# data61/gossamer

Measured on AMD Instinct MI355X. Metric: M k-mers/s (canonical, counted) at k=25, 150 bp reads, higher is better.
Workload: dtype u64

## Files before the change

### gossamer_amd/csrc/fused_path.hpp

```cpp
#pragma once

enum { kFusedDeclined = 0, kFusedDone = 1, kFusedNeedFull = 2, kFusedGoOn = -1, kFusedAgain = -2 };
constexpr uint32_t kFusedGrid = 256 * GOSS_E1_OCC;
#ifndef GOSS_FUSED_NKEYS2
#define GOSS_FUSED_NKEYS2 14
#endif
#ifndef GOSS_FUSED_GRID2
#define GOSS_FUSED_GRID2 512
#endif
constexpr uint32_t kFusedGrid2 = GOSS_FUSED_GRID2;
constexpr double kValidSlackA = 1.06, kValidSlackB = 1.17;
constexpr uint64_t kValidSizingMin = 640u << 20;

struct FusedForm {
    enum Table {
        kSmall,
        kBig,
        kWide,
        k96,
        kRem32
    };
    Table table = kSmall;
    uint32_t segbits = kSegBits;
    bool msd = false;
// ... 516 lines not shown
    out->n = n; out->tiles = tiles; out->windows = hp->windows;
    return kFusedGoOn;
}

struct FusedLookback { LookbackCtl* ctl; LookbackCtl* hctl; };

inline int count_rem32(const FusedChunk<Key1>& ch, FusedForm form, const Sub32Regions& sub, const FirstLevelResult& fl, const GapTable* dgt,
                       FusedLookback lb, Run* r)
{
    goss_gpu_ctx* c = ch.c;
    Key1* ka = ch.ka; Key1* kb = ch.kb;
    const uint64_t n = fl.n, tiles = fl.tiles;
    const uint32_t r32_regions = form.r32_regions(), r32_bits = form.r32_bits, r32_split = form.r32_split, rbits32 = form.rbits32;
    const uint32_t sqbit32 = c->len - 1;
    const bool narrow = form.narrow, squeeze = form.squeeze;
    SubTable32* dsub = (SubTable32*)c->arena.temp(sizeof(SubTable32));
    unsigned long long* cur2 = (unsigned long long*)c->arena.temp((uint64_t)r32_regions * 4);
    uint64_t* seg_beg = (uint64_t*)c->arena.temp((uint64_t)r32_regions * 8);
    uint64_t* seg_end = (uint64_t*)c->arena.temp((uint64_t)r32_regions * 8);
    Tile32* tdesc = (Tile32*)c->arena.temp(std::max<uint64_t>(tiles, 1) * sizeof(Tile32));
    HIP_TRY(hipMemcpyAsync(dsub->start, sub.start.data(), (uint64_t)r32_regions * 8, hipMemcpyHostToDevice, c->stream));
    HIP_TRY(hipMemcpyAsync(dsub->cap, sub.cap.data(), (uint64_t)r32_regions * 4, hipMemcpyHostToDevice, c->stream));
    HIP_TRY(hipMemsetAsync(cur2, 0, (uint64_t)r32_regions * 4, c->stream));
    if (narrow && r32_bits == 9)
        hipLaunchKernelGGL(HIP_KERNEL_NAME(tiles32_kernel<Sub32N<9>::kTileSlots>), dim3(grid_for(tiles, 256)), dim3(256), 0, c->stream,
                           dgt, tdesc, (uint32_t)tiles);
    else if (narrow)
        hipLaunchKernelGGL(HIP_KERNEL_NAME(tiles32_kernel<Sub32N<10>::kTileSlots>), dim3(grid_for(tiles, 256)), dim3(256), 0, c->stream,
                           dgt, tdesc, (uint32_t)tiles);
    else
        hipLaunchKernelGGL(HIP_KERNEL_NAME(tiles32_kernel<kSub32Tile>), dim3(grid_for(tiles, 256)), dim3(256), 0, c->stream,
                           dgt, tdesc, (uint32_t)tiles);
    {
        PhaseTimer t(c, GOSS_T_SCATTER, n);
        const dim3 g2((uint32_t)((tiles + 7) / 8 * 8));
#define GOSS_LAUNCH_S32N(SQ, B2, NRW)                                                                                    \
    hipLaunchKernelGGL(HIP_KERNEL_NAME(subpart32_kernel<SQ, B2, NRW>), g2, dim3(kTB), 0, c->stream, (const Key1*)ka, (uint32_t*)kb, rbits32, \
                       sqbit32, cur2, (const Tile32*)tdesc, (uint32_t)tiles, (const SubTable32*)dsub, lb.ctl)
#define GOSS_LAUNCH_S32(SQ, B2) do { if (narrow) GOSS_LAUNCH_S32N(SQ, B2, true); else GOSS_LAUNCH_S32N(SQ, B2, false); } while (0)
        if (squeeze) GOSS_LAUNCH_S32(true, 9);
        else if (r32_bits == 9) GOSS_LAUNCH_S32(false, 9);
        else GOSS_LAUNCH_S32(false, 10);
#undef GOSS_LAUNCH_S32
#undef GOSS_LAUNCH_S32N
        t.stop();
    }
    hipLaunchKernelGGL(sub_bounds32_kernel, dim3(r32_regions / 256), dim3(256), 0, c->stream, (const SubTable32*)dsub,
                       (const uint32_t*)cur2, r32_regions, seg_beg, seg_end);
    HIP_TRY(hipMemcpyAsync(lb.hctl, lb.ctl, sizeof(LookbackCtl), hipMemcpyDeviceToHost, c->stream));
    HIP_TRY(hipStreamSynchronize(c->stream));
    if (lb.hctl->error) { c->fused_overflows++; return ch.decline("a 32-bit sub-region overflowed"); }
    ch.lap("second level (32-bit remainders)");
    const uint32_t* rems = (const uint32_t*)kb;
    Key1* spare32 = ka;
    uint32_t nseg32 = r32_regions;
    if (r32_split)
    {
        nseg32 = r32_regions << r32_split;
        uint64_t* sub_beg = (uint64_t*)c->arena.temp((uint64_t)nseg32 * 8);
// ... 1 lines not shown
        {
            PhaseTimer t(c, GOSS_T_SCATTER, n);
            hipLaunchKernelGGL(subsplit32_kernel, unit_grid(r32_regions), dim3(kTB), 0, c->stream, (const uint32_t*)kb, (uint32_t*)ka,
                               (const uint64_t*)seg_beg, (const uint64_t*)seg_end, rbits32 - (squeeze ? 1u : 0u), r32_split, sub_beg, sub_end);
            t.stop();
        }
        check_launch("third-level split kernel");
        seg_beg = sub_beg; seg_end = sub_end;
        rems = (const uint32_t*)ka;
        spare32 = kb;
        ch.lap("third level (sub-segments)");
    }
    int rc;
    for (;;)
    {
        rc = segment_reduce32(c, rems, spare32, n, r, seg_beg, seg_end, form.r32_slots, squeeze, rbits32, sqbit32, nseg32, r32_split);
        if (rc != 1 || form.r32_slots >= 16384 || c->rem32_slots) break;
        c->segment_retries++;
        form = form.larger_r32_table();
    }
    if (rc != 0)
    {
        c->segment_retries++;
        if (rc == 1 && r32_split < (uint32_t)kSub32SplitMax) c->rem32_split_min = r32_split + 1;
        else c->rem32 = false;
        if (c->debug) std::fprintf(stderr, "libgossgpu: fused path: 32-bit form with %u + %u bits overflowed (%d), redoing the chunk %s\n", r32_bits, r32_split, rc,
                                   c->rem32 ? "with more sub-segments" : "in the 8-byte form");
        return kFusedAgain;
    }
    c->fused_msd_chunks++;
    c->rem32_chunks++;
// ... 238 lines not shown
```

### gossamer_amd/csrc/goss_gpu.hip

```cpp
#include "../../include/goss_gpu.h"

#include <hip/hip_runtime.h>
#include <dlfcn.h>

#include <algorithm>
#include <chrono>
#include <cmath>
#include <cstdio>
#include <cstdlib>
#include <cstring>
#include <functional>
#include <map>
#include <mutex>
#include <string>
#include <system_error>
#include <thread>
#include <vector>

#include "goss_kernels.hpp"
#include "goss_reader.hpp"

using namespace goss;

namespace {
// ... 1015 lines not shown
    HIP_TRY(hipMemcpyAsync(seg_dst, seg_cnt, (uint64_t)nunit * 8, hipMemcpyDeviceToDevice, c->stream));
    exclusive_scan_u64(c, seg_dst, nunit);
    out->m = m;
    out->keys = c->arena.perm(std::max<uint64_t>(m, 1) * sizeof(K));
    out->counts = (uint32_t*)c->arena.perm(std::max<uint64_t>(m, 1) * 4);
    hipLaunchKernelGGL(HIP_KERNEL_NAME(seg_gather_kernel<K>), unit_grid(nunit), dim3(kTB), 0, c->stream,
                       (const K*)stage_keys, (const uint32_t*)stage_counts, (const uint64_t*)seg_pos,
                       (const uint64_t*)seg_dst, (const uint64_t*)seg_cnt, (K*)out->keys, out->counts);
    t.stop();
    HIP_TRY(hipStreamSynchronize(c->stream));
    c->arena.release(mark);
    return 0;
}

int segment_reduce32(goss_gpu_ctx* c, const uint32_t* rems, Key1* spare, uint64_t n, Run* out, const uint64_t* seg_beg,
                     const uint64_t* seg_end, int slots, bool squeeze, uint32_t rbits, uint32_t sqbit, uint32_t nseg, uint32_t split_bits)
{
    uint64_t mark = c->arena.mark();
    PhaseTimer t(c, GOSS_T_REDUCE, n);
    uint64_t* seg_pos = (uint64_t*)c->arena.temp((uint64_t)nseg * 8);
    uint64_t* seg_cnt = (uint64_t*)c->arena.temp(((uint64_t)nseg + 1) * 8);
    uint64_t* seg_dst = (uint64_t*)c->arena.temp(((uint64_t)nseg + 1) * 8);
    SegOut* so = (SegOut*)c->arena.temp(sizeof(SegOut));
    const uint64_t cap = n * sizeof(Key1) / (sizeof(Key1) + 4);
    Key1* stage_keys = spare;
    uint32_t* stage_counts = (uint32_t*)(spare + cap);
    SegOut hso{};
    hso.stage_cap = cap;
    HIP_TRY(hipMemcpyAsync(so, &hso, sizeof(SegOut), hipMemcpyHostToDevice, c->stream));
#define GOSS_LAUNCH_R32(SLOTS, SQ)                                                                                       \
    hipLaunchKernelGGL(HIP_KERNEL_NAME(seg_hash_reduce32b_kernel<SLOTS, SQ>), unit_grid(nseg), dim3(SLOTS <= 4096 ? kTB : SLOTS / 4096 * kTB), 0, c->stream, rems, seg_beg, \
                       seg_end, so, seg_pos, seg_cnt, stage_keys, stage_counts, rbits, sqbit, split_bits)
    if (slots == 2048) { if (squeeze) GOSS_LAUNCH_R32(2048, true); else GOSS_LAUNCH_R32(2048, false); }
    else if (slots == 8192) { if (squeeze) GOSS_LAUNCH_R32(8192, true); else GOSS_LAUNCH_R32(8192, false); }
    else if (slots == 16384) { if (squeeze) GOSS_LAUNCH_R32(16384, true); else GOSS_LAUNCH_R32(16384, false); }
    else { if (squeeze) GOSS_LAUNCH_R32(4096, true); else GOSS_LAUNCH_R32(4096, false); }
#undef GOSS_LAUNCH_R32
    check_launch("32-bit segment counting kernel");
    SegOut* h = (SegOut*)c->h_pinned;
    HIP_TRY(hipMemcpyAsync(h, so, sizeof(SegOut), hipMemcpyDeviceToHost, c->stream));
    HIP_TRY(hipStreamSynchronize(c->stream));
#if defined(GOSS_STAMPS)
    if (h->stamps[7])
        std::fprintf(stderr, "libgossgpu: counting stamps per segment (cycles of wave 0): set-up %.0f  loads+copy %.0f  fast path %.0f  slow path %.0f  closing barrier %.0f  ordering %.0f  write-out %.0f   (%llu segments)\n",
                     (double)h->stamps[0] / h->stamps[7], (double)h->stamps[1] / h->stamps[7], (double)h->stamps[2] / h->stamps[7], (double)h->stamps[3] / h->stamps[7],
                     (double)h->stamps[4] / h->stamps[7], (double)h->stamps[5] / h->stamps[7], (double)h->stamps[6] / h->stamps[7], (unsigned long long)h->stamps[7]);
#endif
    if (h->overflow == 1u && c->overflow_by_sort)
    {
        SegOut hs = *h;
        const int rc = count_overflowed_units<Key1>(c, nseg, seg_beg, seg_end, seg_pos, seg_cnt, &hs, stage_keys, stage_counts,
            [&](uint32_t u, uint64_t first, uint64_t cnt_u, Key1* dst) {
                const uint64_t prefix = (uint64_t)(u >> split_bits) << rbits;
                if (squeeze)
                    hipLaunchKernelGGL(HIP_KERNEL_NAME(expand_rem32_kernel<true>), dim3(grid_for(cnt_u, kTB)), dim3(kTB), 0, c->stream, rems + first, cnt_u, prefix, sqbit, dst);
                else
                    hipLaunchKernelGGL(HIP_KERNEL_NAME(expand_rem32_kernel<false>), dim3(grid_for(cnt_u, kTB)), dim3(kTB), 0, c->stream, rems + first, cnt_u, prefix, sqbit, dst);
            },
            [&](uint32_t u) -> Key1 {
                const uint32_t rem_bits = rbits - (squeeze ? 1u : 0u);
                const uint32_t sub = split_bits ? (u & ((1u << split_bits) - 1u)) << (rem_bits - split_bits) : 0u;
                const uint64_t low = squeeze ? rem32_unpack<true>(sub, sqbit) : rem32_unpack<false>(sub, sqbit);
                return Key1{((uint64_t)(u >> split_bits) << rbits) | low};
            });
        *h = hs;
        if (rc == 2) h->overflow = 2u;
    }
    if (h->overflow)
    {
        const int why = (h->overflow & 1u) ? 1 : 2;
        t.stop();
        c->arena.release(mark);
// ... 3988 lines not shown
```

### gossamer_amd/csrc/kernels_count.hpp

```cpp
#pragma once
#include <type_traits>

#include <hip/hip_runtime.h>
#include <stdint.h>

#include "goss_key.hpp"
#include "kernels_partition.hpp"

namespace goss {


constexpr int kSegBits = 16;
constexpr int kSegBitsMax = 24;
constexpr int kSegSlots = 4096;
constexpr int kSegLimit = 3072;
constexpr int kSegSlots2 = 2048;
constexpr int kSegLimit2 = 1536;

template <class K>
__global__ void seg_bounds_kernel(const K* __restrict__ keys, uint64_t n, uint32_t shift, uint32_t nseg,
                                  uint64_t* __restrict__ seg_off)
{
    uint32_t s = blockIdx.x * blockDim.x + threadIdx.x;
    if (s > nseg) return;
// ... 6 lines not shown
    seg_off[s] = a;
}

struct SegOut {
    unsigned long long cursor;
    uint32_t overflow;
    uint32_t count_overflow;
    unsigned long long stage_cap;
#if defined(GOSS_STAMPS)
    unsigned long long stamps[8];
#endif
};

constexpr unsigned long long kSegOverflowed = ~0ULL;

template <bool SQ>
__global__ __launch_bounds__(kTB) void expand_rem32_kernel(const uint32_t* __restrict__ rems, uint64_t n, uint64_t prefix, uint32_t sqbit,
                                                           Key1* __restrict__ out)
{
    const uint64_t i = (uint64_t)blockIdx.x * kTB + threadIdx.x;
    if (i < n) out[i].lo = prefix | rem32_unpack<SQ>(rems[i], sqbit);
}
__global__ __launch_bounds__(kTB) void expand_rem96_kernel(const Rem96* __restrict__ recs, uint64_t n, uint64_t seg, uint32_t rem_bits,
                                                           Key2* __restrict__ out)
{
    const uint64_t i = (uint64_t)blockIdx.x * kTB + threadIdx.x;
    if (i >= n) return;
    const Rem96 r = recs[i];
    const unsigned __int128 full = ((unsigned __int128)seg << rem_bits) | ((unsigned __int128)r.r2 << 64) | ((uint64_t)r.r0 | ((uint64_t)r.r1 << 32));
    out[i] = Key2{(uint64_t)full, (uint64_t)(full >> 64)};
}

template <class K>
__global__ __launch_bounds__(kTB) void unit_bounds_kernel(const K* __restrict__ keys, uint64_t m, const K* __restrict__ lows, const K* __restrict__ highs,
                                                          const uint8_t* __restrict__ last, const uint32_t* __restrict__ units, uint32_t nunits,
                                                          unsigned long long cursor, uint64_t* __restrict__ seg_pos, uint64_t* __restrict__ seg_cnt)
// ... 433 lines not shown
                                                                             uint32_t rem_bits, uint32_t round_bits)
{
    (void)round_bits;
    seg_hash_reduce_body<kSegBigThreads, kSegBigSlots, false>(keys, seg_off, seg_end, so, seg_pos, seg_cnt, stage_keys, stage_counts, rem_bits, 0u);
}

__global__ __launch_bounds__(kSegBigThreads) void seg_hash_reduce_shared_kernel(const Key1* __restrict__ keys, const uint64_t* __restrict__ seg_off,
                                                                                const uint64_t* __restrict__ seg_end, SegOut* __restrict__ so,
                                                                                uint64_t* __restrict__ seg_pos, uint64_t* __restrict__ seg_cnt,
                                                                                Key1* __restrict__ stage_keys, uint32_t* __restrict__ stage_counts,
                                                                                uint32_t rem_bits, uint32_t round_bits)
{
    seg_hash_reduce_body<kSegBigThreads, kSegBigSlots, true>(keys, seg_off, seg_end, so, seg_pos, seg_cnt, stage_keys, stage_counts, rem_bits, round_bits);
}

constexpr uint32_t kR32Mul = 0x9E3779B1u, kR32MulInv = 0x0E8B2F51u;
__host__ __device__ __forceinline__ uint32_t r32_mix(uint32_t k) { return (k ^ (k >> 15)) * kR32Mul; }
__host__ __device__ __forceinline__ uint32_t r32_unmix(uint32_t f) { const uint32_t y = f * kR32MulInv; return y ^ (y >> 15) ^ (y >> 30); }

__device__ __forceinline__ uint32_t r32b_slot_offset(const uint32_t __attribute__((ext_vector_type(4)))& q, uint32_t k)
{
    uint32_t off;
    unsigned long long m0, m1, m2, m3;
    asm("v_cmp_eq_u32_e64 %1, %5, %9\n\t"
        "v_cmp_eq_u32_e64 %2, %6, %9\n\t"
        "v_cmp_eq_u32_e64 %3, %7, %9\n\t"
        "v_cmp_eq_u32_e64 %4, %8, %9\n\t"
        "v_cndmask_b32_e64 %0, 16, 12, %1\n\t"
        "v_cndmask_b32_e64 %0, %0, 8, %2\n\t"
        "v_cndmask_b32_e64 %0, %0, 4, %3\n\t"
        "v_cndmask_b32_e64 %0, %0, 0, %4"
        : "=&v"(off), "=&s"(m0), "=&s"(m1), "=&s"(m2), "=&s"(m3)
        : "v"(q.w), "v"(q.z), "v"(q.y), "v"(q.x), "v"(k));
// ... 8 lines not shown
        "v_cmp_lt_u32_e64 %6, 15, %10\n\t"
        "v_cmp_lt_u32_e64 %7, 15, %11\n\t"
        "v_cndmask_b32_e64 %0, %0, %12, %4\n\t"
        "v_cndmask_b32_e64 %1, %1, %12, %5\n\t"
        "v_cndmask_b32_e64 %2, %2, %12, %6\n\t"
        "v_cndmask_b32_e64 %3, %3, %12, %7"
        : "+v"(t[0]), "+v"(t[1]), "+v"(t[2]), "+v"(t[3]), "=&s"(m0), "=&s"(m1), "=&s"(m2), "=&s"(m3)
        : "v"(off[0]), "v"(off[1]), "v"(off[2]), "v"(off[3]), "v"(dummy));
}

#ifndef GOSS_R32B_VEC
#define GOSS_R32B_VEC 4
#endif
template <int SLOTS> struct R32bCfg { static constexpr int kThreads = SLOTS <= 4096 ? kTB : SLOTS == 8192 ? 2 * kTB : 4 * kTB;
                                      static constexpr int kOcc = SLOTS == 2048 ? 5 : SLOTS == 4096 ? 4 : SLOTS == 8192 ? 2 : 1; };
template <int SLOTS, bool SQ>
__global__ __launch_bounds__(R32bCfg<SLOTS>::kThreads, R32bCfg<SLOTS>::kOcc) void seg_hash_reduce32b_kernel(const uint32_t* __restrict__ rems, const uint64_t* __restrict__ seg_off,
                                                                const uint64_t* __restrict__ seg_end, SegOut* __restrict__ so,
                                                                uint64_t* __restrict__ seg_pos, uint64_t* __restrict__ seg_cnt,
                                                                Key1* __restrict__ stage_keys, uint32_t* __restrict__ stage_counts,
                                                                uint32_t rbits, uint32_t sqbit, uint32_t split_bits)
{
    constexpr int NT = R32bCfg<SLOTS>::kThreads;
    constexpr int kLimit = SLOTS / 4 * 3;
    constexpr int BB = SLOTS == 16384 ? 12 : SLOTS == 8192 ? 11 : SLOTS == 4096 ? 10 : SLOTS == 2048 ? 9 : -1;
    constexpr uint32_t NB = SLOTS / 4;
    constexpr uint32_t kCnt = 4u * SLOTS;
    static_assert(BB > 0, "table size");
    __shared__ __attribute__((aligned(16))) unsigned long long tab[SLOTS + 32];
    __shared__ uint32_t ndist, ovf;
    __shared__ unsigned long long sh_base;
// ... 11 lines not shown
        return;
    }
    if (e - b > 0xFFFFFFF0ULL)
    {
        if (tid == 0) { atomicOr(&so->overflow, 2u); seg_pos[s] = 0; seg_cnt[s] = 0; }
        return;
    }
    typedef uint32_t u32x4 __attribute__((ext_vector_type(4)));
    typedef __attribute__((address_space(3))) uint8_t* lds_bytes;
    typedef const __attribute__((address_space(3))) u32x4* lds_bucket_plain;
    typedef const volatile __attribute__((address_space(3))) u32x4* lds_bucket_ptr;
    typedef __attribute__((address_space(3))) uint32_t* lds_word;
    const lds_bytes tb = (lds_bytes)tab;
    uint32_t* const tkey = reinterpret_cast<uint32_t*>(tab);
    uint32_t* const tcnt = tkey + SLOTS;
    auto marker = [](uint32_t bkt) -> uint32_t { return r32_unmix(((bkt ^ 1u) << (32 - BB)) | (3u << (32 - 2 * BB))); };
    for (uint32_t i = tid; i < NB; i += NT)
    {
        const uint32_t m = marker(i);
        *(__attribute__((address_space(3))) u32x4*)(tb + 16 * i) = u32x4{m, m, m, m};
        *(__attribute__((address_space(3))) u32x4*)(tb + kCnt + 16 * i) = u32x4{0u, 0u, 0u, 0u};
    }
    if (tid < 32) tab[SLOTS + tid] = 0;
    if (tid == 0) { ndist = 0; ovf = 0; }
    __syncthreads();
    GOSS_STAMP(0);

    lds_vu32 vovf = (lds_vu32)&ovf;
    const uint32_t dummy = 8u * (uint32_t)SLOTS + 4u * (tid & 63u);
    auto home_of = [](uint32_t f) -> uint32_t { return f >> (32 - BB); };
    auto second_of = [](uint32_t f, uint32_t h) -> uint32_t { return h ^ (((f >> (32 - 2 * BB)) & (NB - 1u)) | 1u); };

    constexpr int kVec = GOSS_R32B_VEC;
    const uint32_t head = (uint32_t)(b & 3ULL);
    const u32x4* const v4 = reinterpret_cast<const u32x4*>(rems + (b - head));
    const uint32_t n = (uint32_t)(e - b) + head;
    const uint32_t nvec = (n + 3u) >> 2, nfull = n >> 2;
    u32x4 nxt[kVec];
#pragma unroll
    for (int u = 0; u < kVec; ++u)
    {
        const uint32_t i = (uint32_t)u * NT + tid;
        nxt[u] = __builtin_nontemporal_load(&v4[i < nvec ? i : nvec - 1]);
    }
    for (uint32_t i0 = 0; i0 < nvec; i0 += (uint32_t)NT * kVec)
    {
// ... 3 lines not shown
#pragma unroll
        for (int u = 0; u < kVec; ++u)
        {
            const uint32_t i = i0 + (uint32_t)(kVec + u) * NT + tid;
            nxt[u] = __builtin_nontemporal_load(&v4[i < nvec ? i : nvec - 1]);
        }
        GOSS_STAMP(1);
        auto four_keys = [&](const u32x4& v, uint32_t live, auto whole_tag) -> uint32_t {
            constexpr bool kWhole = decltype(whole_tag)::value;
            const uint32_t kk[4] = {v.x, v.y, v.z, v.w};
            uint32_t f[4], a1[4], off[4];
            u32x4 q[4];
#pragma unroll
            for (int j = 0; j < 4; ++j)
            {
                f[j] = r32_mix(kk[j]);
                a1[j] = home_of(f[j]) << 4;
                q[j] = *(lds_bucket_plain)(tb + a1[j]);
            }
#pragma unroll
            for (int j = 0; j < 4; ++j) off[j] = r32b_slot_offset(q[j], kk[j]);
            uint32_t t[4];
#pragma unroll
            for (int j = 0; j < 4; ++j)
            {
                t[j] = kCnt + a1[j] + off[j];
                bool miss = off[j] == 16u;
                if (!kWhole) miss = miss && ((live >> j) & 1u);
                if (__builtin_expect(__ballot(miss) != 0, 0))
                {
                    if (miss)
                    {
// ... 17 lines not shown
                __hip_atomic_fetch_add((lds_word)(tb + t[j]), 1u, __ATOMIC_RELAXED, __HIP_MEMORY_SCOPE_WORKGROUP);
                left |= (off[j] & 16u) << j;
            }
            return left >> 4;
        };
        auto slow_keys = [&](const u32x4& v, uint32_t pd) {
            uint32_t key = 0, bk = 0, f = 0, st = 0, moves = 0;
            bool busy = false;
            for (;;)
            {
                if (!busy && pd)
                {
                    const uint32_t j = __ffs(pd) - 1;
                    pd &= pd - 1;
                    key = j == 0 ? v.x : j == 1 ? v.y : j == 2 ? v.z : v.w;
                    f = r32_mix(key);
                    bk = home_of(f);
                    st = 0;
                    busy = true;
                }
                if (!__ballot(busy)) break;
                if (busy)
                {
                    const u32x4 q = *(lds_bucket_ptr)(tb + 16u * bk);
                    const uint32_t mk = marker(bk);
                    const u32x4 qq = u32x4{q.x, q.y, q.z, q.w};
                    const uint32_t ho = r32b_slot_offset(qq, key);
                    const uint32_t eo = r32b_slot_offset(qq, mk);
                    uint32_t hit = ~0u;
                    if (key != mk && ho < 16u) hit = 4 * bk + (ho >> 2);
                    else if (key != mk && eo < 16u)
                    {
// ... 43 lines not shown
    __syncthreads();
    GOSS_STAMP(4);
    if (ovf)
    {
        if (tid == 0) { atomicOr(&so->overflow, 1u); seg_pos[s] = 0; seg_cnt[s] = kSegOverflowed; }
        return;
    }

    constexpr int kPer = SLOTS / NT;
    constexpr int kBins = SLOTS / 4, kBinsPer = kBins / NT, kBinBits = BB;
    __shared__ uint32_t bins[kBins];
    __shared__ uint32_t sh_scan2[NT / 64 + 1];
    __shared__ uint32_t big;
    unsigned long long ck[kPer];
#pragma unroll
    for (int j = 0; j < kPer; ++j) ck[j] = ((unsigned long long)tcnt[tid * kPer + j] << 32) | tkey[tid * kPer + j];
    for (uint32_t i = tid; i < kBins; i += NT) bins[i] = 0;
    if (tid == 0) big = 0;
    __syncthreads();
    const uint32_t rem_bits = rbits - (SQ ? 1u : 0u);
    const uint32_t bsh = rem_bits > (uint32_t)kBinBits + split_bits ? rem_bits - split_bits - kBinBits : 0;
    uint32_t rnk[kPer];
#pragma unroll
    for (int j = 0; j < kPer; ++j)
        if ((ck[j] >> 32) != 0) rnk[j] = atomicAdd(&bins[((uint32_t)ck[j] >> bsh) & (kBins - 1)], 1u);
    __syncthreads();
    uint32_t bn[kBinsPer], bs[kBinsPer], mine = 0;
#pragma unroll
    for (int q = 0; q < kBinsPer; ++q) { bn[q] = bins[tid * kBinsPer + q]; mine += bn[q]; }
    uint32_t tot_occ;
    uint32_t at = block_excl_scan_n<uint32_t, NT / 64>(mine, sh_scan2, &tot_occ);
// ... 737 lines not shown
```

### gossamer_amd/csrc/kernels_extract.hpp

```cpp
#pragma once
#include <type_traits>

#include <hip/hip_runtime.h>
#include <stdint.h>

#include "goss_key.hpp"
#include "kernels_common.hpp"

namespace goss {


struct ExtractCounters {
    unsigned long long keys_out;
    unsigned long long windows;
    unsigned long long hist[512];
};

template <bool PACKED = false>
__global__ __launch_bounds__(kTB) void nonbase_sample_kernel(const uint8_t* __restrict__ aligned, uint64_t nslices,
                                                             uint64_t stride, uint32_t slice,
                                                             unsigned long long* __restrict__ out)
{
    unsigned long long bad = 0, seen = 0;
    for (uint64_t s = blockIdx.x; s < nslices; s += gridDim.x)
// ... 784 lines not shown
                    if (MODE == 0 && REPK == 1)
                    {
                        const uint32_t sel = (uint32_t)__builtin_amdgcn_sbfe((int32_t)flo, len - 1u, 1u);
                        kreg[i].lo = ((uint64_t)bit_select(sel, rhi, fhi) << 32) | bit_select(sel, rlo, flo);
                    }
                    else emit(i, ((uint64_t)fhi << 32) | flo, ((uint64_t)rhi << 32) | rlo);
                    if (i + 1 < P)
                    {
                        r_s2 += 2u;
                        if (r_s2 >= r_nw2 && r_at < 511) next_rec();
                    }
                }
            }
            else if constexpr (FAST)
            {
                const uint32_t kmhi = (uint32_t)(kmask >> 32);
                const uint32_t cw0 = ~(uint32_t)blo, cw1 = ~(uint32_t)(blo >> 32), cw2 = ~(uint32_t)bhi;
                const uint32_t pn = bits - 2;
                const uint32_t nx = (uint32_t)((blo >> pn) | (bhi << (64 - pn)));
                const uint32_t mid = (uint32_t)(blo >> (len - 1));
                const uint64_t f0 = rev64(blo & kmask) >> (64 - bits);
                uint32_t flo = (uint32_t)f0, fhi = (uint32_t)(f0 >> 32);
#pragma unroll
                for (int i = 0; i < P; ++i)
                {
                    if (i)
                    {
                        const uint32_t nb = (nx >> (2 * i)) & 3u;
                        fhi = __builtin_amdgcn_alignbit(fhi, flo, 30) & kmhi;
                        flo = (flo << 2) | nb;
                    }
                    const uint32_t rlo = i ? __builtin_amdgcn_alignbit(cw1, cw0, 2 * i) : cw0;
                    const uint32_t rhi = (i ? __builtin_amdgcn_alignbit(cw2, cw1, 2 * i) : cw1) & kmhi;
                    if (MODE == 0 && REPK == 1)
                    {
                        const uint32_t sel = (uint32_t)__builtin_amdgcn_sbfe((int32_t)mid, 2 * i, 1);
                        kreg[i].lo = ((uint64_t)bit_select(sel, rhi, fhi) << 32) | bit_select(sel, rlo, flo);
                    }
                    else emit(i, ((uint64_t)fhi << 32) | flo, ((uint64_t)rhi << 32) | rlo);
#pragma unroll
                    for (int u = 0; u < S; ++u) rank_key(i * S + u);
                }
            }
            else
            {
                uint64_t f = rev64(blo & kmask) >> (64 - bits);
                uint64_t r = (~blo) & kmask;
                const uint32_t top = bits - 2;
// ... 153 lines not shown
#endif
        {
            uint32_t tb[NK];
#pragma unroll
            for (int i = 0; i < NK; ++i) tb[i] = *reinterpret_cast<const uint32_t*>(reinterpret_cast<const char*>(tab) + bin4[i]);
            if constexpr (NARROW)
            {
                auto put = [&](auto sq_tag, auto hi_tag) {
                    constexpr bool kSq = decltype(sq_tag)::value, kHi = decltype(hi_tag)::value;
                    const uint32_t lomask = kSq ? (1u << nr_sqbit) - 1u : (nr_rbits >= 32 ? 0xFFFFFFFFu : (1u << nr_rbits) - 1u);
                    const uint32_t dbits = (uint32_t)__popc(nr_dmask);
#pragma unroll
                    for (int i = 0; i < NK; ++i)
                    {
                        const uint32_t klo = (uint32_t)kreg[i].lo, khi = (uint32_t)(kreg[i].lo >> 32);
                        uint32_t rem = klo & lomask;
                        if (kSq) rem |= __builtin_amdgcn_alignbit(khi, klo, nr_sqbit + 1u) << nr_sqbit;
                        const uint32_t dg = kHi ? __builtin_amdgcn_ubfe(khi, nr_rbits - 32u, dbits)
                                                : (__builtin_amdgcn_alignbit(khi, klo, nr_rbits) & nr_dmask);
                        const uint32_t la = tb[i] + (rk[i] << 2);
                        *reinterpret_cast<uint32_t*>(lds_all + la) = rem;
                        *reinterpret_cast<uint16_t*>(lds_all + kDigBase + (la >> 1)) = (uint16_t)dg;
                    }
                };
                if (nr_sqbit) { if (nr_rbits >= 32) put(std::true_type{}, std::true_type{}); else put(std::true_type{}, std::false_type{}); }
                else { if (nr_rbits >= 32) put(std::false_type{}, std::true_type{}); else put(std::false_type{}, std::false_type{}); }
            }
            else
#pragma unroll
            for (int i = 0; i < NK; ++i)
            {
                *reinterpret_cast<Key1*>(reinterpret_cast<char*>(sorted) + (tb[i] + (rk[i] << 3))) = kreg[i];
                if (NH > 0)
                {
// ... 736 lines not shown
```

### gossamer_amd/csrc/kernels_partition.hpp

```cpp
#pragma once

#include <hip/hip_runtime.h>
#include <stdint.h>

#include "goss_key.hpp"
#include "kernels_common.hpp"

namespace goss {


#ifndef GOSS_SORT_ITEMS1
#define GOSS_SORT_ITEMS1 32
#endif
#ifndef GOSS_SORT_ITEMS2
#define GOSS_SORT_ITEMS2 16
#endif
#ifndef GOSS_LB_BATCH
#define GOSS_LB_BATCH 1
#endif
template <class K> struct SubCfg {
    static constexpr int kItems = sizeof(K) == 8 ? 22 : 11;
    static constexpr int kTile = 256 * kItems;
};

// ... 458 lines not shown
        K k = stage[i];
        uint64_t o = global_base[key_digit(k, digit)] + i;
        keys_out[o] = k;
        if (HAS_VAL) vals_out[o] = vstage[i];
    }
}

constexpr int kSub32BitsMin = 9, kSub32BitsMax = 10;
constexpr int kSub32SplitMax = 4;
constexpr uint32_t kSub32RegionsMax = 256u << kSub32BitsMax;
struct SubTable32 {
    unsigned long long start[kSub32RegionsMax];
    uint32_t cap[kSub32RegionsMax];
};

template <bool SQ>
__host__ __device__ __forceinline__ uint32_t rem32_pack(uint64_t key, uint32_t rbits, uint32_t sqbit)
{
    const uint64_t x = key & ((1ULL << rbits) - 1ULL);
    if (!SQ) return (uint32_t)x;
    return (uint32_t)(((x >> (sqbit + 1)) << sqbit) | (x & ((1ULL << sqbit) - 1ULL)));
}
template <bool SQ>
__host__ __device__ __forceinline__ uint64_t rem32_unpack(uint32_t r, uint32_t sqbit)
{
    if (!SQ) return r;
    return (((uint64_t)r >> sqbit) << (sqbit + 1)) | ((uint64_t)r & ((1ULL << sqbit) - 1ULL));
}

struct Tile32 { unsigned long long base; uint32_t n, bucket; };
#ifndef GOSS_S32_ITEMS
#define GOSS_S32_ITEMS 22
#endif
constexpr int kSub32Items = GOSS_S32_ITEMS;
constexpr int kSub32Tile = kTB * kSub32Items;
template <int TILE>
__global__ void tiles32_kernel(const GapTable* __restrict__ gt, Tile32* __restrict__ desc, uint32_t total)
{
    const uint32_t t = blockIdx.x * blockDim.x + threadIdx.x;
    if (t >= total) return;
    uint32_t lo = 0, hi = 255;
    while (lo < hi)
    {
// ... 1 lines not shown
        if (gt->tile_first[mid] <= t) lo = mid; else hi = mid - 1;
    }
    const uint64_t j = (uint64_t)t - gt->tile_first[lo];
    const uint64_t left = gt->cnt[lo] - j * TILE;
    desc[t] = Tile32{gt->reg_start[lo] + j * TILE, (uint32_t)(left < (uint64_t)TILE ? left : (uint64_t)TILE), lo};
}

#ifndef GOSS_S32_OCC
#define GOSS_S32_OCC 4
#endif
#ifndef GOSS_S32_CH
#define GOSS_S32_CH 10
#define GOSS_S32_OCCN 3
#endif
template <int B2> struct Sub32N { static constexpr int kChunks = B2 == 9 ? GOSS_S32_CH : GOSS_S32_CH - 1; static constexpr int kTileSlots = kTB * kChunks * 2; };
template <bool SQ, int B2, bool NARROW = false>
__global__ __launch_bounds__(kTB, NARROW ? GOSS_S32_OCCN : GOSS_S32_OCC) void subpart32_kernel(const Key1* __restrict__ keys_in, uint32_t* __restrict__ out,
                                                           uint32_t rbits, uint32_t sqbit, unsigned long long* __restrict__ cursors,
                                                           const Tile32* __restrict__ desc, uint32_t total_tiles,
                                                           const SubTable32* __restrict__ sub, LookbackCtl* __restrict__ ctl)
{
    constexpr int kSub32ChunksN = Sub32N<B2>::kChunks;
    constexpr int kItems = NARROW ? 3 * kSub32ChunksN : kSub32Items;
    static_assert(NARROW || kItems <= 32, "one bit of `have` per key");
    constexpr int kTile = kTB * kItems;
    constexpr uint32_t ND = 1u << B2;
    constexpr int DPT = ND / kTB;
    static_assert(DPT >= 2 && DPT % 2 == 0, "a thread owns pairs of digits");
    __shared__ uint32_t stage[kTile];
    __shared__ uint16_t sdig[kTile];
    __shared__ uint32_t hist[ND];
    __shared__ uint32_t gbase[ND];
    __shared__ uint32_t sh_scan[kWaves + 1];
    __shared__ uint32_t sh_skip, sh_total;

    const uint32_t tid = threadIdx.x, lane = lane_id(), w = wave_id();
    const uint32_t per = (total_tiles + 7u) / 8u;
    const uint32_t tile = (blockIdx.x & 7u) * per + (blockIdx.x >> 3);
    if (tile >= total_tiles) return;
    const Tile32 td = desc[tile];
    const uint32_t b = td.bucket, tile_n = td.n;
    const uint64_t tile_base = td.base;
    if (tid == 0) sh_skip = 0;
#pragma unroll
    for (int j = 0; j < DPT; ++j) hist[tid + j * kTB] = 0;

    __builtin_amdgcn_s_setprio(3);
    Key1 key[NARROW ? 1 : kItems];
    [[maybe_unused]] uint32_t rem[NARROW ? kItems : 1], dw[NARROW ? kSub32ChunksN : 1];
    uint16_t rank[kItems];
    uint32_t have = 0;
    const uint32_t wbase = w * 64 * kItems;
    if constexpr (NARROW)
    {
        const uint32_t nchunk = tile_n >> 1;
        const uint4* const cin = reinterpret_cast<const uint4*>(keys_in + tile_base);
        const uint32_t cbase = w * 64 * kSub32ChunksN;
#pragma unroll
        for (int r = 0; r < kSub32ChunksN; ++r)
        {
            const uint32_t ci = cbase + r * 64 + lane;
            dw[r] = 0;
            rem[3 * r] = rem[3 * r + 1] = rem[3 * r + 2] = 0;
            if (ci < nchunk)
            {
                const uint4 v = cin[ci];
                rem[3 * r] = v.x; rem[3 * r + 1] = v.y; rem[3 * r + 2] = v.z; dw[r] = v.w;
            }
        }
        __builtin_amdgcn_s_setprio(0);
        __syncthreads();
#pragma unroll
        for (int r = 0; r < kItems; ++r)
            if ((dw[r / 3] >> 30) > (uint32_t)(r % 3)) rank[r] = (uint16_t)atomicAdd(&hist[(dw[r / 3] >> (10 * (r % 3))) & (ND - 1u)], 1u);
    }
    else
    {
#if !defined(GOSS_S32_LOAD8)
    static_assert(kItems % 2 == 0, "pairs of keys per load");
#pragma unroll
    for (int r = 0; r < kItems / 2; ++r)
    {
        const uint32_t li = wbase + r * 128 + 2 * lane;
        if (li < tile_n)
        {
#if defined(GOSS_S32_NT)
            typedef uint32_t u32x4_ __attribute__((ext_vector_type(4)));
            const u32x4_ vv = __builtin_nontemporal_load(reinterpret_cast<const u32x4_*>(keys_in + tile_base + li));
            const uint4 v = make_uint4(vv.x, vv.y, vv.z, vv.w);
// ... 45 lines not shown
        for (int j = 0; j < DPT; ++j)
        {
            hist[DPT * tid + j] = start;
            gbase[DPT * tid + j] = (mine ? (uint32_t)(sub->start[sidx + j] - region_first) : 0u) + ex[j] - start;
            start += cn[j];
        }
        if (tid == 0) sh_total = tile_total;
    }
    __syncthreads();
#pragma unroll
    for (int r = 0; r < kItems; ++r)
        if (NARROW ? (dw[NARROW ? r / 3 : 0] >> 30) > (uint32_t)(r % 3) : ((have >> (r & 31)) & 1u) != 0)
        {
            if constexpr (NARROW)
            {
                const uint32_t d = (dw[r / 3] >> (10 * (r % 3))) & (ND - 1u);
                const uint32_t at = hist[d] + rank[r];
                stage[at] = rem[r];
                sdig[at] = (uint16_t)d;
            }
            else
            {
            const uint32_t d = (uint32_t)(key[r].lo >> rbits) & (ND - 1u);
            const uint32_t at = hist[d] + rank[r];
            stage[at] = rem32_pack<SQ>(key[r].lo, rbits, sqbit);
            sdig[at] = (uint16_t)d;
            }
        }
    __syncthreads();
    if (sh_skip) return;
    const uint32_t tile_keys = sh_total;
    uint32_t* const out_r = out + region_first;
    for (uint32_t i = tid; i < tile_keys; i += kTB)
    {
#if defined(GOSS_S32_EXP) && GOSS_S32_EXP == 1
        asm volatile("" ::"v"(gbase[sdig[i]]), "v"(stage[i]));
#else
        out_r[(uint32_t)(gbase[sdig[i]] + i)] = stage[i];
#endif
    }
// ... 122 lines not shown
```

Measured before the change: 179,900.

## Store pre-mixed hash images of 32-bit remainders so the reduce skips rehashing

When no third-level split is used, the second-level scatter now writes each 32-bit remainder as its rotated mixed hash image instead of the raw value. The segment hash-reduce kernel then takes the bucket index straight from the stored word, so it no longer rehashes every key. The original remainder is recovered with an inverse mix only at output and expansion time. The change also makes the extraction kernel emit the raw 10-bit field for the narrow squeeze form and defers the squeeze repacking to the scatter, and it drops a mask in the loose narrow extraction path. It adds more template instantiations and makes correctness depend on the mix being exactly invertible.

```diff
diff --git a/gossamer_amd/csrc/fused_path.hpp b/gossamer_amd/csrc/fused_path.hpp
--- a/gossamer_amd/csrc/fused_path.hpp
+++ b/gossamer_amd/csrc/fused_path.hpp
@@ -554,6 +554,9 @@
     const uint32_t r32_regions = form.r32_regions(), r32_bits = form.r32_bits, r32_split = form.r32_split, rbits32 = form.rbits32;
     const uint32_t sqbit32 = c->len - 1;
     const bool narrow = form.narrow, squeeze = form.squeeze;
+    const bool image = r32_split == 0;
+    if (squeeze && (rbits32 != kNarrowSqRbits || r32_bits != kNarrowSqDigitBits))
+        throw StatusError{GOSS_ERR_HIP, "fused path: the squeeze form with other than 33-bit remainders under nine second-level bits"};
     SubTable32* dsub = (SubTable32*)c->arena.temp(sizeof(SubTable32));
     unsigned long long* cur2 = (unsigned long long*)c->arena.temp((uint64_t)r32_regions * 4);
     uint64_t* seg_beg = (uint64_t*)c->arena.temp((uint64_t)r32_regions * 8);
@@ -574,15 +577,17 @@
     {
         PhaseTimer t(c, GOSS_T_SCATTER, n);
         const dim3 g2((uint32_t)((tiles + 7) / 8 * 8));
-#define GOSS_LAUNCH_S32N(SQ, B2, NRW)                                                                                    \
-    hipLaunchKernelGGL(HIP_KERNEL_NAME(subpart32_kernel<SQ, B2, NRW>), g2, dim3(kTB), 0, c->stream, (const Key1*)ka, (uint32_t*)kb, rbits32, \
+#define GOSS_LAUNCH_S32I(SQ, B2, NRW, IMG)                                                                               \
+    hipLaunchKernelGGL(HIP_KERNEL_NAME(subpart32_kernel<SQ, B2, NRW, IMG>), g2, dim3(kTB), 0, c->stream, (const Key1*)ka, (uint32_t*)kb, rbits32, \
                        sqbit32, cur2, (const Tile32*)tdesc, (uint32_t)tiles, (const SubTable32*)dsub, lb.ctl)
+#define GOSS_LAUNCH_S32N(SQ, B2, NRW) do { if (image) GOSS_LAUNCH_S32I(SQ, B2, NRW, true); else GOSS_LAUNCH_S32I(SQ, B2, NRW, false); } while (0)
 #define GOSS_LAUNCH_S32(SQ, B2) do { if (narrow) GOSS_LAUNCH_S32N(SQ, B2, true); else GOSS_LAUNCH_S32N(SQ, B2, false); } while (0)
         if (squeeze) GOSS_LAUNCH_S32(true, 9);
         else if (r32_bits == 9) GOSS_LAUNCH_S32(false, 9);
         else GOSS_LAUNCH_S32(false, 10);
 #undef GOSS_LAUNCH_S32
 #undef GOSS_LAUNCH_S32N
+#undef GOSS_LAUNCH_S32I
         t.stop();
     }
     hipLaunchKernelGGL(sub_bounds32_kernel, dim3(r32_regions / 256), dim3(256), 0, c->stream, (const SubTable32*)dsub,
@@ -614,7 +619,7 @@
     int rc;
     for (;;)
     {
-        rc = segment_reduce32(c, rems, spare32, n, r, seg_beg, seg_end, form.r32_slots, squeeze, rbits32, sqbit32, nseg32, r32_split);
+        rc = segment_reduce32(c, rems, spare32, n, r, seg_beg, seg_end, form.r32_slots, squeeze, image, rbits32, sqbit32, nseg32, r32_split);
         if (rc != 1 || form.r32_slots >= 16384 || c->rem32_slots) break;
         c->segment_retries++;
         form = form.larger_r32_table();
diff --git a/gossamer_amd/csrc/goss_gpu.hip b/gossamer_amd/csrc/goss_gpu.hip
--- a/gossamer_amd/csrc/goss_gpu.hip
+++ b/gossamer_amd/csrc/goss_gpu.hip
@@ -1053,7 +1053,7 @@
 }
 
 int segment_reduce32(goss_gpu_ctx* c, const uint32_t* rems, Key1* spare, uint64_t n, Run* out, const uint64_t* seg_beg,
-                     const uint64_t* seg_end, int slots, bool squeeze, uint32_t rbits, uint32_t sqbit, uint32_t nseg, uint32_t split_bits)
+                     const uint64_t* seg_end, int slots, bool squeeze, bool image, uint32_t rbits, uint32_t sqbit, uint32_t nseg, uint32_t split_bits)
 {
     uint64_t mark = c->arena.mark();
     PhaseTimer t(c, GOSS_T_REDUCE, n);
@@ -1067,14 +1067,16 @@
     SegOut hso{};
     hso.stage_cap = cap;
     HIP_TRY(hipMemcpyAsync(so, &hso, sizeof(SegOut), hipMemcpyHostToDevice, c->stream));
-#define GOSS_LAUNCH_R32(SLOTS, SQ)                                                                                       \
-    hipLaunchKernelGGL(HIP_KERNEL_NAME(seg_hash_reduce32b_kernel<SLOTS, SQ>), unit_grid(nseg), dim3(SLOTS <= 4096 ? kTB : SLOTS / 4096 * kTB), 0, c->stream, rems, seg_beg, \
+#define GOSS_LAUNCH_R32I(SLOTS, SQ, IMG)                                                                                 \
+    hipLaunchKernelGGL(HIP_KERNEL_NAME(seg_hash_reduce32b_kernel<SLOTS, SQ, IMG>), unit_grid(nseg), dim3(SLOTS <= 4096 ? kTB : SLOTS / 4096 * kTB), 0, c->stream, rems, seg_beg, \
                        seg_end, so, seg_pos, seg_cnt, stage_keys, stage_counts, rbits, sqbit, split_bits)
+#define GOSS_LAUNCH_R32(SLOTS, SQ) do { if (image) GOSS_LAUNCH_R32I(SLOTS, SQ, true); else GOSS_LAUNCH_R32I(SLOTS, SQ, false); } while (0)
     if (slots == 2048) { if (squeeze) GOSS_LAUNCH_R32(2048, true); else GOSS_LAUNCH_R32(2048, false); }
     else if (slots == 8192) { if (squeeze) GOSS_LAUNCH_R32(8192, true); else GOSS_LAUNCH_R32(8192, false); }
     else if (slots == 16384) { if (squeeze) GOSS_LAUNCH_R32(16384, true); else GOSS_LAUNCH_R32(16384, false); }
     else { if (squeeze) GOSS_LAUNCH_R32(4096, true); else GOSS_LAUNCH_R32(4096, false); }
 #undef GOSS_LAUNCH_R32
+#undef GOSS_LAUNCH_R32I
     check_launch("32-bit segment counting kernel");
     SegOut* h = (SegOut*)c->h_pinned;
     HIP_TRY(hipMemcpyAsync(h, so, sizeof(SegOut), hipMemcpyDeviceToHost, c->stream));
@@ -1091,10 +1093,11 @@
         const int rc = count_overflowed_units<Key1>(c, nseg, seg_beg, seg_end, seg_pos, seg_cnt, &hs, stage_keys, stage_counts,
             [&](uint32_t u, uint64_t first, uint64_t cnt_u, Key1* dst) {
                 const uint64_t prefix = (uint64_t)(u >> split_bits) << rbits;
-                if (squeeze)
-                    hipLaunchKernelGGL(HIP_KERNEL_NAME(expand_rem32_kernel<true>), dim3(grid_for(cnt_u, kTB)), dim3(kTB), 0, c->stream, rems + first, cnt_u, prefix, sqbit, dst);
-                else
-                    hipLaunchKernelGGL(HIP_KERNEL_NAME(expand_rem32_kernel<false>), dim3(grid_for(cnt_u, kTB)), dim3(kTB), 0, c->stream, rems + first, cnt_u, prefix, sqbit, dst);
+#define GOSS_LAUNCH_X32(SQ, IMG)                                                                                         \
+    hipLaunchKernelGGL(HIP_KERNEL_NAME(expand_rem32_kernel<SQ, IMG>), dim3(grid_for(cnt_u, kTB)), dim3(kTB), 0, c->stream, rems + first, cnt_u, prefix, sqbit, dst)
+                if (squeeze) { if (image) GOSS_LAUNCH_X32(true, true); else GOSS_LAUNCH_X32(true, false); }
+                else { if (image) GOSS_LAUNCH_X32(false, true); else GOSS_LAUNCH_X32(false, false); }
+#undef GOSS_LAUNCH_X32
             },
             [&](uint32_t u) -> Key1 {
                 const uint32_t rem_bits = rbits - (squeeze ? 1u : 0u);
diff --git a/gossamer_amd/csrc/goss_words.hpp b/gossamer_amd/csrc/goss_words.hpp
--- /dev/null
+++ b/gossamer_amd/csrc/goss_words.hpp
@@ -0,0 +1,58 @@
+#pragma once
+#include <cstdint>
+
+#if defined(__HIPCC__)
+#define GOSS_HD __host__ __device__ __forceinline__
+#else
+#define GOSS_HD inline
+#endif
+
+namespace goss {
+
+template <bool SQ>
+GOSS_HD uint32_t rem32_pack(uint64_t key, uint32_t rbits, uint32_t sqbit)
+{
+    const uint64_t x = key & ((1ULL << rbits) - 1ULL);
+    if (!SQ) return (uint32_t)x;
+    return (uint32_t)(((x >> (sqbit + 1)) << sqbit) | (x & ((1ULL << sqbit) - 1ULL)));
+}
+template <bool SQ>
+GOSS_HD uint64_t rem32_unpack(uint32_t r, uint32_t sqbit)
+{
+    if (!SQ) return r;
+    return (((uint64_t)r >> sqbit) << (sqbit + 1)) | ((uint64_t)r & ((1ULL << sqbit) - 1ULL));
+}
+
+GOSS_HD uint32_t funnel_shr(uint32_t hi, uint32_t lo, uint32_t s)
+{
+#if defined(__HIP_DEVICE_COMPILE__)
+    return __builtin_amdgcn_alignbit(hi, lo, s);
+#else
+    return (uint32_t)((((uint64_t)hi << 32) | lo) >> s);
+#endif
+}
+
+constexpr uint32_t kNarrowSqRbits = 33, kNarrowSqDigitBits = 9;
+GOSS_HD uint32_t narrow_sq_field(uint32_t key_hi) { return key_hi & 0x3FFu; }
+GOSS_HD uint32_t narrow_sq_digit(uint32_t field) { return (field >> 1) & ((1u << kNarrowSqDigitBits) - 1u); }
+GOSS_HD uint32_t narrow_sq_rem(uint32_t key_lo, uint32_t field, uint32_t sqbit)
+{
+    return (key_lo & ((1u << sqbit) - 1u)) | (funnel_shr(field, key_lo, sqbit + 1u) << sqbit);
+}
+
+constexpr uint32_t kR32Mul = 0x9E3779B1u, kR32MulInv = 0x0E8B2F51u;
+GOSS_HD uint32_t r32_mix(uint32_t k) { return (k ^ (k >> 15)) * kR32Mul; }
+GOSS_HD uint32_t r32_unmix(uint32_t f) { const uint32_t y = f * kR32MulInv; return y ^ (y >> 15) ^ (y >> 30); }
+
+GOSS_HD uint32_t r32_image(uint32_t k) { const uint32_t f = r32_mix(k); return (f >> 16) | (f << 16); }
+GOSS_HD uint32_t r32_unimage(uint32_t w) { return r32_unmix((w >> 16) | (w << 16)); }
+GOSS_HD uint32_t r32_image_home_bytes(uint32_t w, uint32_t nb) { return w & ((nb - 1u) << 4); }
+GOSS_HD uint32_t r32_image_home(uint32_t w, uint32_t nb) { return (w >> 4) & (nb - 1u); }
+GOSS_HD uint32_t r32_image_second(uint32_t w, uint32_t home, uint32_t nb) { return home ^ (((w >> 20) & (nb - 1u)) | 1u); }
+GOSS_HD uint32_t r32_image_marker(uint32_t bkt) { return ((bkt ^ 1u) << 4) | (3u << 20); }
+
+GOSS_HD uint32_t r32_plain_home(uint32_t f, uint32_t bb) { return f >> (32u - bb); }
+GOSS_HD uint32_t r32_plain_second(uint32_t f, uint32_t home, uint32_t bb) { return home ^ (((f >> (32u - 2u * bb)) & ((1u << bb) - 1u)) | 1u); }
+GOSS_HD uint32_t r32_plain_marker(uint32_t bkt, uint32_t bb) { return r32_unmix(((bkt ^ 1u) << (32u - bb)) | (3u << (32u - 2u * bb))); }
+
+}
diff --git a/gossamer_amd/csrc/kernels_count.hpp b/gossamer_amd/csrc/kernels_count.hpp
--- a/gossamer_amd/csrc/kernels_count.hpp
+++ b/gossamer_amd/csrc/kernels_count.hpp
@@ -44,12 +44,12 @@
 
 constexpr unsigned long long kSegOverflowed = ~0ULL;
 
-template <bool SQ>
+template <bool SQ, bool IMG = false>
 __global__ __launch_bounds__(kTB) void expand_rem32_kernel(const uint32_t* __restrict__ rems, uint64_t n, uint64_t prefix, uint32_t sqbit,
                                                            Key1* __restrict__ out)
 {
     const uint64_t i = (uint64_t)blockIdx.x * kTB + threadIdx.x;
-    if (i < n) out[i].lo = prefix | rem32_unpack<SQ>(rems[i], sqbit);
+    if (i < n) out[i].lo = prefix | rem32_unpack<SQ>(IMG ? r32_unimage(rems[i]) : rems[i], sqbit);
 }
 __global__ __launch_bounds__(kTB) void expand_rem96_kernel(const Rem96* __restrict__ recs, uint64_t n, uint64_t seg, uint32_t rem_bits,
                                                            Key2* __restrict__ out)
@@ -513,9 +513,6 @@
     seg_hash_reduce_body<kSegBigThreads, kSegBigSlots, true>(keys, seg_off, seg_end, so, seg_pos, seg_cnt, stage_keys, stage_counts, rem_bits, round_bits);
 }
 
-constexpr uint32_t kR32Mul = 0x9E3779B1u, kR32MulInv = 0x0E8B2F51u;
-__host__ __device__ __forceinline__ uint32_t r32_mix(uint32_t k) { return (k ^ (k >> 15)) * kR32Mul; }
-__host__ __device__ __forceinline__ uint32_t r32_unmix(uint32_t f) { const uint32_t y = f * kR32MulInv; return y ^ (y >> 15) ^ (y >> 30); }
 
 __device__ __forceinline__ uint32_t r32b_slot_offset(const uint32_t __attribute__((ext_vector_type(4)))& q, uint32_t k)
 {
@@ -554,7 +551,7 @@
 #endif
 template <int SLOTS> struct R32bCfg { static constexpr int kThreads = SLOTS <= 4096 ? kTB : SLOTS == 8192 ? 2 * kTB : 4 * kTB;
                                       static constexpr int kOcc = SLOTS == 2048 ? 5 : SLOTS == 4096 ? 4 : SLOTS == 8192 ? 2 : 1; };
-template <int SLOTS, bool SQ>
+template <int SLOTS, bool SQ, bool IMG = false>
 __global__ __launch_bounds__(R32bCfg<SLOTS>::kThreads, R32bCfg<SLOTS>::kOcc) void seg_hash_reduce32b_kernel(const uint32_t* __restrict__ rems, const uint64_t* __restrict__ seg_off,
                                                                 const uint64_t* __restrict__ seg_end, SegOut* __restrict__ so,
                                                                 uint64_t* __restrict__ seg_pos, uint64_t* __restrict__ seg_cnt,
@@ -596,7 +593,7 @@
     const lds_bytes tb = (lds_bytes)tab;
     uint32_t* const tkey = reinterpret_cast<uint32_t*>(tab);
     uint32_t* const tcnt = tkey + SLOTS;
-    auto marker = [](uint32_t bkt) -> uint32_t { return r32_unmix(((bkt ^ 1u) << (32 - BB)) | (3u << (32 - 2 * BB))); };
+    auto marker = [](uint32_t bkt) -> uint32_t { return IMG ? r32_image_marker(bkt) : r32_plain_marker(bkt, BB); };
     for (uint32_t i = tid; i < NB; i += NT)
     {
         const uint32_t m = marker(i);
@@ -610,8 +607,9 @@
 
     lds_vu32 vovf = (lds_vu32)&ovf;
     const uint32_t dummy = 8u * (uint32_t)SLOTS + 4u * (tid & 63u);
-    auto home_of = [](uint32_t f) -> uint32_t { return f >> (32 - BB); };
-    auto second_of = [](uint32_t f, uint32_t h) -> uint32_t { return h ^ (((f >> (32 - 2 * BB)) & (NB - 1u)) | 1u); };
+    auto f_of = [](uint32_t word) -> uint32_t { return IMG ? word : r32_mix(word); };
+    auto home16_of = [](uint32_t f) -> uint32_t { return IMG ? r32_image_home_bytes(f, NB) : r32_plain_home(f, BB) << 4; };
+    auto second_of = [](uint32_t f, uint32_t h) -> uint32_t { return IMG ? r32_image_second(f, h, NB) : r32_plain_second(f, h, BB); };
 
     constexpr int kVec = GOSS_R32B_VEC;
     const uint32_t head = (uint32_t)(b & 3ULL);
@@ -645,8 +643,8 @@
 #pragma unroll
             for (int j = 0; j < 4; ++j)
             {
-                f[j] = r32_mix(kk[j]);
-                a1[j] = home_of(f[j]) << 4;
+                f[j] = f_of(kk[j]);
+                a1[j] = home16_of(f[j]);
                 q[j] = *(lds_bucket_plain)(tb + a1[j]);
             }
 #pragma unroll
@@ -694,8 +692,8 @@
                     const uint32_t j = __ffs(pd) - 1;
                     pd &= pd - 1;
                     key = j == 0 ? v.x : j == 1 ? v.y : j == 2 ? v.z : v.w;
-                    f = r32_mix(key);
-                    bk = home_of(f);
+                    f = f_of(key);
+                    bk = home16_of(f) >> 4;
                     st = 0;
                     busy = true;
                 }
@@ -769,7 +767,11 @@
     __shared__ uint32_t big;
     unsigned long long ck[kPer];
 #pragma unroll
-    for (int j = 0; j < kPer; ++j) ck[j] = ((unsigned long long)tcnt[tid * kPer + j] << 32) | tkey[tid * kPer + j];
+    for (int j = 0; j < kPer; ++j)
+    {
+        const uint32_t word = tkey[tid * kPer + j];
+        ck[j] = ((unsigned long long)tcnt[tid * kPer + j] << 32) | (IMG ? r32_unimage(word) : word);
+    }
     for (uint32_t i = tid; i < kBins; i += NT) bins[i] = 0;
     if (tid == 0) big = 0;
     __syncthreads();
diff --git a/gossamer_amd/csrc/kernels_extract.hpp b/gossamer_amd/csrc/kernels_extract.hpp
--- a/gossamer_amd/csrc/kernels_extract.hpp
+++ b/gossamer_amd/csrc/kernels_extract.hpp
@@ -6,6 +6,7 @@
 
 #include "goss_key.hpp"
 #include "kernels_common.hpp"
+#include "goss_words.hpp"
 
 namespace goss {
 
@@ -822,7 +823,8 @@
             }
             else if constexpr (FAST)
             {
-                const uint32_t kmhi = (uint32_t)(kmask >> 32);
+                constexpr bool kLoose = MODE == 0 && REPK == 1 && NARROW && NH == 0;
+                [[maybe_unused]] const uint32_t kmhi = (uint32_t)(kmask >> 32);
                 const uint32_t cw0 = ~(uint32_t)blo, cw1 = ~(uint32_t)(blo >> 32), cw2 = ~(uint32_t)bhi;
                 const uint32_t pn = bits - 2;
                 const uint32_t nx = (uint32_t)((blo >> pn) | (bhi << (64 - pn)));
@@ -835,11 +837,13 @@
                     if (i)
                     {
                         const uint32_t nb = (nx >> (2 * i)) & 3u;
-                        fhi = __builtin_amdgcn_alignbit(fhi, flo, 30) & kmhi;
+                        fhi = __builtin_amdgcn_alignbit(fhi, flo, 30);
+                        if constexpr (!kLoose) fhi &= kmhi;
                         flo = (flo << 2) | nb;
                     }
                     const uint32_t rlo = i ? __builtin_amdgcn_alignbit(cw1, cw0, 2 * i) : cw0;
-                    const uint32_t rhi = (i ? __builtin_amdgcn_alignbit(cw2, cw1, 2 * i) : cw1) & kmhi;
+                    uint32_t rhi = i ? __builtin_amdgcn_alignbit(cw2, cw1, 2 * i) : cw1;
+                    if constexpr (!kLoose) rhi &= kmhi;
                     if (MODE == 0 && REPK == 1)
                     {
                         const uint32_t sel = (uint32_t)__builtin_amdgcn_sbfe((int32_t)mid, 2 * i, 1);
@@ -1023,10 +1027,19 @@
                     for (int i = 0; i < NK; ++i)
                     {
                         const uint32_t klo = (uint32_t)kreg[i].lo, khi = (uint32_t)(kreg[i].lo >> 32);
-                        uint32_t rem = klo & lomask;
-                        if (kSq) rem |= __builtin_amdgcn_alignbit(khi, klo, nr_sqbit + 1u) << nr_sqbit;
-                        const uint32_t dg = kHi ? __builtin_amdgcn_ubfe(khi, nr_rbits - 32u, dbits)
-                                                : (__builtin_amdgcn_alignbit(khi, klo, nr_rbits) & nr_dmask);
+                        uint32_t rem, dg;
+                        if constexpr (kSq && kHi)
+                        {
+                            rem = klo;
+                            dg = narrow_sq_field(khi);
+                        }
+                        else
+                        {
+                            rem = klo & lomask;
+                            if (kSq) rem |= __builtin_amdgcn_alignbit(khi, klo, nr_sqbit + 1u) << nr_sqbit;
+                            dg = kHi ? __builtin_amdgcn_ubfe(khi, nr_rbits - 32u, dbits)
+                                     : (__builtin_amdgcn_alignbit(khi, klo, nr_rbits) & nr_dmask);
+                        }
                         const uint32_t la = tb[i] + (rk[i] << 2);
                         *reinterpret_cast<uint32_t*>(lds_all + la) = rem;
                         *reinterpret_cast<uint16_t*>(lds_all + kDigBase + (la >> 1)) = (uint16_t)dg;
diff --git a/gossamer_amd/csrc/kernels_partition.hpp b/gossamer_amd/csrc/kernels_partition.hpp
--- a/gossamer_amd/csrc/kernels_partition.hpp
+++ b/gossamer_amd/csrc/kernels_partition.hpp
@@ -5,6 +5,7 @@
 
 #include "goss_key.hpp"
 #include "kernels_common.hpp"
+#include "goss_words.hpp"
 
 namespace goss {
 
@@ -496,19 +497,6 @@
     uint32_t cap[kSub32RegionsMax];
 };
 
-template <bool SQ>
-__host__ __device__ __forceinline__ uint32_t rem32_pack(uint64_t key, uint32_t rbits, uint32_t sqbit)
-{
-    const uint64_t x = key & ((1ULL << rbits) - 1ULL);
-    if (!SQ) return (uint32_t)x;
-    return (uint32_t)(((x >> (sqbit + 1)) << sqbit) | (x & ((1ULL << sqbit) - 1ULL)));
-}
-template <bool SQ>
-__host__ __device__ __forceinline__ uint64_t rem32_unpack(uint32_t r, uint32_t sqbit)
-{
-    if (!SQ) return r;
-    return (((uint64_t)r >> sqbit) << (sqbit + 1)) | ((uint64_t)r & ((1ULL << sqbit) - 1ULL));
-}
 
 struct Tile32 { unsigned long long base; uint32_t n, bucket; };
 #ifndef GOSS_S32_ITEMS
@@ -540,12 +528,13 @@
 #define GOSS_S32_OCCN 3
 #endif
 template <int B2> struct Sub32N { static constexpr int kChunks = B2 == 9 ? GOSS_S32_CH : GOSS_S32_CH - 1; static constexpr int kTileSlots = kTB * kChunks * 2; };
-template <bool SQ, int B2, bool NARROW = false>
+template <bool SQ, int B2, bool NARROW = false, bool IMG = false>
 __global__ __launch_bounds__(kTB, NARROW ? GOSS_S32_OCCN : GOSS_S32_OCC) void subpart32_kernel(const Key1* __restrict__ keys_in, uint32_t* __restrict__ out,
                                                            uint32_t rbits, uint32_t sqbit, unsigned long long* __restrict__ cursors,
                                                            const Tile32* __restrict__ desc, uint32_t total_tiles,
                                                            const SubTable32* __restrict__ sub, LookbackCtl* __restrict__ ctl)
 {
+    static_assert(!SQ || B2 == (int)kNarrowSqDigitBits, "the squeeze form has nine second-level bits");
     constexpr int kSub32ChunksN = Sub32N<B2>::kChunks;
     constexpr int kItems = NARROW ? 3 * kSub32ChunksN : kSub32Items;
     static_assert(NARROW || kItems <= 32, "one bit of `have` per key");
@@ -572,6 +561,7 @@
     for (int j = 0; j < DPT; ++j) hist[tid + j * kTB] = 0;
 
     __builtin_amdgcn_s_setprio(3);
+    [[maybe_unused]] auto field_digit = [](uint32_t field) -> uint32_t { return SQ ? narrow_sq_digit(field) : field & (ND - 1u); };
     Key1 key[NARROW ? 1 : kItems];
     [[maybe_unused]] uint32_t rem[NARROW ? kItems : 1], dw[NARROW ? kSub32ChunksN : 1];
     uint16_t rank[kItems];
@@ -598,7 +588,7 @@
         __syncthreads();
 #pragma unroll
         for (int r = 0; r < kItems; ++r)
-            if ((dw[r / 3] >> 30) > (uint32_t)(r % 3)) rank[r] = (uint16_t)atomicAdd(&hist[(dw[r / 3] >> (10 * (r % 3))) & (ND - 1u)], 1u);
+            if ((dw[r / 3] >> 30) > (uint32_t)(r % 3)) rank[r] = (uint16_t)atomicAdd(&hist[field_digit(dw[r / 3] >> (10 * (r % 3)))], 1u);
     }
     else
     {
@@ -674,16 +664,19 @@
         {
             if constexpr (NARROW)
             {
-                const uint32_t d = (dw[r / 3] >> (10 * (r % 3))) & (ND - 1u);
+                const uint32_t field = dw[r / 3] >> (10 * (r % 3));
+                const uint32_t d = field_digit(field);
                 const uint32_t at = hist[d] + rank[r];
-                stage[at] = rem[r];
+                const uint32_t word = SQ ? narrow_sq_rem(rem[r], field, sqbit) : rem[r];
+                stage[at] = IMG ? r32_image(word) : word;
                 sdig[at] = (uint16_t)d;
             }
             else
             {
             const uint32_t d = (uint32_t)(key[r].lo >> rbits) & (ND - 1u);
             const uint32_t at = hist[d] + rank[r];
-            stage[at] = rem32_pack<SQ>(key[r].lo, rbits, sqbit);
+            const uint32_t word = rem32_pack<SQ>(key[r].lo, rbits, sqbit);
+            stage[at] = IMG ? r32_image(word) : word;
             sdig[at] = (uint16_t)d;
             }
         }
```

Result: faster. 182,600 (median of 6 runs) (+1.5%).
